# CloudEngineHub/FairyGen

Hardware: AMD Instinct MI355X
Metric: decoded frames/sec (sec/clip in config), Wan2.2-TI2V-5B 704x1280x121 @ 5 steps (higher is better)
Workload: dtype bf16

## Files before the change

### fairygen_amd/csrc/dit_elementwise.hip

```cpp
#include "common.h"
#include "rmsnorm_rope_row.h"

#ifndef FG_ROW_MIN_WAVES
#define FG_ROW_MIN_WAVES 4
#endif
#define FG_ROW_BOUNDS __launch_bounds__(256, FG_ROW_MIN_WAVES)

namespace {

__device__ __forceinline__ void row_moments(const Row& r, int C, int lane, float eps, float& mean, float& rstd) {
    const int nvec = C >> 3;
    float s = 0.f;
#pragma unroll
    for (int i = 0; i < kMaxVec; ++i)
#pragma unroll
        for (int j = 0; j < 8; ++j) s += r.v[i][j];
    mean = wave_sum(s) / (float)C;
    float q = 0.f;
#pragma unroll
    for (int i = 0; i < kMaxVec; ++i) {
        if (lane + i * 64 < nvec) {
#pragma unroll
            for (int j = 0; j < 8; ++j) {
                const float d = r.v[i][j] - mean;
                q += d * d;
            }
        }
    }
    const float var = wave_sum(q) / (float)C;
    rstd = 1.0f / sqrtf(var + eps);
}

__device__ __forceinline__ int64_t mod_row(int64_t row, int64_t mod_rows, int64_t first_rows) {
    return mod_rows == 1 ? 0 : (mod_rows == 2 ? (row < first_rows ? 0 : 1) : row);
}

template <int MODE>
__device__ __forceinline__ void norm_store(const Row& r, int C, int lane, float eps, const bf16* p0, const bf16* p1,
                                           bf16* out) {
    const int nvec = C >> 3;
    float mean, rstd;
    row_moments(r, C, lane, eps, mean, rstd);
#pragma unroll
    for (int i = 0; i < kMaxVec; ++i) {
        const int vi = lane + i * 64;
        if (vi < nvec) {
            const bf16x8 a = ld8(p0 + (int64_t)vi * 8);
            const bf16x8 b = ld8(p1 + (int64_t)vi * 8);
            float o[8];
#pragma unroll
            for (int j = 0; j < 8; ++j) {
                const float n = (r.v[i][j] - mean) * rstd;
                if (MODE == 0) {
                    const float y = rbf(n);
                    const float s1 = rbf(1.0f + (float)b[j]);
                    o[j] = rbf(y * s1) + (float)a[j];
                } else {
                    o[j] = n * (float)a[j] + (float)b[j];
                }
            }
            st8(out + (int64_t)vi * 8, o);
        }
    }
}

__device__ __forceinline__ uint32_t cvt2_fp8(float a, float b) {
    return (uint32_t)__builtin_amdgcn_cvt_pk_fp8_f32(a, b, 0, false) & 0xffffu;
}

template <int MODE, bool DUAL = false>
__device__ __forceinline__ void norm_store_fp8(Row& r, int C, int lane, float eps, const bf16* p0, const bf16* p1,
                                               uint8_t* out8, float* scale_out, float fp8_max, bf16* out16 = nullptr) {
    const int nvec = C >> 3;
    float mean, rstd;
    row_moments(r, C, lane, eps, mean, rstd);
    float amax = 0.f;
#pragma unroll
    for (int i = 0; i < kMaxVec; ++i) {
        const int vi = lane + i * 64;
        if (vi < nvec) {
            const bf16x8 a = ld8(p0 + (int64_t)vi * 8);
            const bf16x8 b = ld8(p1 + (int64_t)vi * 8);
#pragma unroll
            for (int j = 0; j < 8; ++j) {
                const float n = (r.v[i][j] - mean) * rstd;
                float o;
                if (MODE == 0) {
                    const float y = rbf(n);
                    const float s1 = rbf(1.0f + (float)b[j]);
                    o = rbf(y * s1) + (float)a[j];
                } else {
                    o = n * (float)a[j] + (float)b[j];
                }
                r.v[i][j] = rbf(o);
                amax = fmaxf(amax, fabsf(r.v[i][j]));
            }
            if (DUAL) st8(out16 + (int64_t)vi * 8, r.v[i]);
        }
    }
    amax = wave_max(amax);
    const float sc = fmaxf(rbf(amax / fp8_max), 1.0f);
    const float denom = sc + 1e-8f;
    if (lane == 0) *scale_out = sc;
#pragma unroll
    for (int i = 0; i < kMaxVec; ++i) {
        const int vi = lane + i * 64;
        if (vi < nvec) {
            u32x2 w;
            w[0] = cvt2_fp8(r.v[i][0] / denom, r.v[i][1] / denom) | (cvt2_fp8(r.v[i][2] / denom, r.v[i][3] / denom) << 16);
            w[1] = cvt2_fp8(r.v[i][4] / denom, r.v[i][5] / denom) | (cvt2_fp8(r.v[i][6] / denom, r.v[i][7] / denom) << 16);
            *reinterpret_cast<u32x2*>(out8 + (int64_t)vi * 8) = w;
        }
    }
}

__global__ FG_ROW_BOUNDS void ln_modulate_fp8_kernel(const bf16* __restrict__ x, const bf16* __restrict__ shift,
                                                     const bf16* __restrict__ scale, uint8_t* __restrict__ out8,
                                                     float* __restrict__ scale_out, int64_t rows, int C, float eps, int64_t mod_rows,
                                                     int64_t first_rows, int64_t mod_ld, float fp8_max) {
    const int lane = threadIdx.x & 63;
    const int64_t row = (int64_t)blockIdx.x * kRowsPerBlock + (threadIdx.x >> 6);
    if (row >= rows) return;
    Row r;
    load_row(x + row * C, C, lane, r);
    const int64_t m = mod_row(row, mod_rows, first_rows);
    norm_store_fp8<0>(r, C, lane, eps, shift + m * mod_ld, scale + m * mod_ld, out8 + row * C, scale_out + row, fp8_max);
}

template <int MODE>
__global__ FG_ROW_BOUNDS void ln_dual_kernel(const bf16* __restrict__ x, const bf16* __restrict__ p0, const bf16* __restrict__ p1,
                                             bf16* __restrict__ out, uint8_t* __restrict__ out8, float* __restrict__ scale_out,
                                             int64_t rows, int C, float eps, int64_t mod_rows, int64_t first_rows, int64_t mod_ld,
                                             float fp8_max) {
    const int lane = threadIdx.x & 63;
    const int64_t row = (int64_t)blockIdx.x * kRowsPerBlock + (threadIdx.x >> 6);
    if (row >= rows) return;
    Row r;
    load_row(x + row * C, C, lane, r);
    const int64_t m = MODE == 0 ? mod_row(row, mod_rows, first_rows) : 0;
    norm_store_fp8<MODE, true>(r, C, lane, eps, p0 + m * mod_ld, p1 + m * mod_ld, out8 + row * C, scale_out + row, fp8_max, out + row * C);
}

__global__ FG_ROW_BOUNDS void ln_modulate_kernel(const bf16* __restrict__ x, const bf16* __restrict__ shift,
                                                          const bf16* __restrict__ scale, bf16* __restrict__ out,
                                                          int64_t rows, int C, float eps, int64_t mod_rows,
                                                          int64_t first_rows, int64_t mod_ld) {
    const int lane = threadIdx.x & 63;
    const int64_t row = (int64_t)blockIdx.x * kRowsPerBlock + (threadIdx.x >> 6);
    if (row >= rows) return;
    Row r;
    load_row(x + row * C, C, lane, r);
    const int64_t m = mod_row(row, mod_rows, first_rows);
    norm_store<0>(r, C, lane, eps, shift + m * mod_ld, scale + m * mod_ld, out + row * C);
}

__global__ FG_ROW_BOUNDS void ln_affine_kernel(const bf16* __restrict__ x, const bf16* __restrict__ w,
                                                        const bf16* __restrict__ b, bf16* __restrict__ out,
                                                        int64_t rows, int C, float eps) {
    const int lane = threadIdx.x & 63;
    const int64_t row = (int64_t)blockIdx.x * kRowsPerBlock + (threadIdx.x >> 6);
    if (row >= rows) return;
    Row r;
    load_row(x + row * C, C, lane, r);
    norm_store<1>(r, C, lane, eps, w, b, out + row * C);
}

template <int MODE>
__global__ FG_ROW_BOUNDS void residual_kernel(const bf16* __restrict__ x, const bf16* __restrict__ y,
                                                       const bf16* __restrict__ gate, bf16* __restrict__ x_out,
                                                       const bf16* __restrict__ p0, const bf16* __restrict__ p1,
                                                       bf16* __restrict__ norm_out, int64_t rows, int C, float eps,
                                                       int64_t mod_rows, int64_t first_rows, int64_t mod_ld,
                                                       uint8_t* __restrict__ norm_fp8 = nullptr, float* __restrict__ norm_scale = nullptr,
                                                       float fp8_max = 0.f) {
    const int lane = threadIdx.x & 63;
    const int64_t row = (int64_t)blockIdx.x * kRowsPerBlock + (threadIdx.x >> 6);
    if (row >= rows) return;
    const int nvec = C >> 3;
    const int64_t m = mod_row(row, mod_rows, first_rows);
    Row r;
#pragma unroll
    for (int i = 0; i < kMaxVec; ++i) {
        const int vi = lane + i * 64;
        if (vi < nvec) {
            const bf16x8 xv = ld8(x + row * C + (int64_t)vi * 8);
            const bf16x8 yv = ld8(y + row * C + (int64_t)vi * 8);
            if (gate != nullptr) {
                const bf16x8 gv = ld8(gate + m * mod_ld + (int64_t)vi * 8);
#pragma unroll
                for (int j = 0; j < 8; ++j) r.v[i][j] = rbf((float)xv[j] + rbf((float)gv[j] * (float)yv[j]));
            } else {
#pragma unroll
                for (int j = 0; j < 8; ++j) r.v[i][j] = rbf((float)xv[j] + (float)yv[j]);
            }
            st8(x_out + row * C + (int64_t)vi * 8, r.v[i]);
        } else {
#pragma unroll
            for (int j = 0; j < 8; ++j) r.v[i][j] = 0.f;
        }
    }
    if (norm_fp8 != nullptr) {
        if (MODE == 0) norm_store_fp8<0>(r, C, lane, eps, p0 + m * mod_ld, p1 + m * mod_ld, norm_fp8 + row * C, norm_scale + row, fp8_max);
        if (MODE == 1) norm_store_fp8<1>(r, C, lane, eps, p0, p1, norm_fp8 + row * C, norm_scale + row, fp8_max);
        return;
    }
    if (MODE == 0) norm_store<0>(r, C, lane, eps, p0 + m * mod_ld, p1 + m * mod_ld, norm_out + row * C);
    if (MODE == 1) norm_store<1>(r, C, lane, eps, p0, p1, norm_out + row * C);
}

template <bool F32TAB, bool PLAIN = false>
__global__ FG_ROW_BOUNDS void rmsnorm_rope_kernel(const bf16* __restrict__ x, int64_t ldx,
                                                           const bf16* __restrict__ w, const void* __restrict__ ctv,
                                                           const void* __restrict__ stv, bf16* __restrict__ out,
                                                           int64_t rows, int C, int head_dim, float eps, int group_cols,
                                                           int64_t out_group_stride, int64_t out_ld) {
    const int lane = threadIdx.x & 63;
    const int64_t row = (int64_t)blockIdx.x * kRowsPerBlock + (threadIdx.x >> 6);
    if (row >= rows) return;
    Row r;
    load_row(x + row * ldx, C, lane, r);
    const int nvec = C >> 3;
    const RopeRow rr = rope_begin<F32TAB, PLAIN>(r, ctv, row, C, head_dim, eps, lane);
#pragma unroll
    for (int i = 0; i < kMaxVec; ++i) {
        const int vi = lane + i * 64;
        if (vi < nvec) {
            float o[8];
            rope_vec<F32TAB, PLAIN>(rr, r.v[i], ld8(w + (int64_t)vi * 8), ctv, stv, row, head_dim, vi, o);
            const int col = vi * 8, g = PLAIN ? 0 : col / group_cols;
            st8(out + g * out_group_stride + row * out_ld + (col - g * group_cols), o);
        }
    }
}

__global__ __launch_bounds__(256) void copy_groups_kernel(const bf16* __restrict__ src, int64_t sgs, int64_t sld,
                                                          bf16* __restrict__ dst, int64_t dgs, int64_t dld, int groups,
                                                          int64_t rows, int vec_per_row) {
    const int64_t total = (int64_t)groups * rows * vec_per_row;
    for (int64_t i = (int64_t)blockIdx.x * blockDim.x + threadIdx.x; i < total; i += (int64_t)gridDim.x * blockDim.x) {
        const int64_t rg = i / vec_per_row;
        const int v = (int)(i - rg * vec_per_row);
        const int64_t r = rg / groups;
        const int g = (int)(rg - r * groups);
        *reinterpret_cast<u32x4*>(dst + g * dgs + r * dld + v * 8) =
            *reinterpret_cast<const u32x4*>(src + g * sgs + r * sld + v * 8);
    }
}


template <int KIND>
__global__ __launch_bounds__(256) void act_kernel(const bf16* __restrict__ x, bf16* __restrict__ out, int64_t nvec) {
    for (int64_t i = (int64_t)blockIdx.x * blockDim.x + threadIdx.x; i < nvec; i += (int64_t)gridDim.x * blockDim.x) {
        const bf16x8 v = ld8(x + i * 8);
        float o[8];
#pragma unroll
        for (int j = 0; j < 8; ++j) o[j] = KIND == 0 ? silu_f((float)v[j]) : gelu_tanh_f((float)v[j]);
        st8(out + i * 8, o);
    }
}

__device__ __forceinline__ float cfg_euler_one(float lat, float p, float ng, bool has_nega, float cfg, float dsigma) {
    const float pred = has_nega ? rbf(ng + rbf(cfg * rbf(p - ng))) : p;
    return rbf(lat + rbf(pred * dsigma));
}

__global__ __launch_bounds__(256) void cfg_euler_kernel(const bf16* __restrict__ lat, const bf16* __restrict__ posi,
                                                        const bf16* __restrict__ nega, bf16* __restrict__ out,
                                                        int64_t n, float cfg, float dsigma) {
    for (int64_t i = (int64_t)blockIdx.x * blockDim.x + threadIdx.x; i < n; i += (int64_t)gridDim.x * blockDim.x)
        out[i] = (bf16)cfg_euler_one((float)lat[i], (float)posi[i], nega != nullptr ? (float)nega[i] : 0.0f, nega != nullptr, cfg, dsigma);
}

__global__ __launch_bounds__(256) void cfg_euler_dev_kernel(const bf16* lat, const bf16* __restrict__ posi, const bf16* __restrict__ nega,
                                                            bf16* out, int64_t n, int64_t nvec, float cfg,
                                                            const float* __restrict__ dsigma_table, const int* __restrict__ step,
                                                            const bf16* __restrict__ first, int64_t first_n, int64_t frame_stride) {
    const float dsigma = dsigma_table[*step];
    const bool has_nega = nega != nullptr;
    const int64_t tid = (int64_t)blockIdx.x * blockDim.x + threadIdx.x, nthreads = (int64_t)gridDim.x * blockDim.x;
    for (int64_t i = tid; i < nvec; i += nthreads) {
        const bf16x8 l = ld8(lat + i * 8), p = ld8(posi + i * 8);
        const bf16x8 g = has_nega ? ld8(nega + i * 8) : p;
        float o[8];
#pragma unroll
        for (int j = 0; j < 8; ++j) o[j] = cfg_euler_one((float)l[j], (float)p[j], (float)g[j], has_nega, cfg, dsigma);
        if (first != nullptr) {
            int64_t ch = (i * 8) / frame_stride, r = i * 8 - ch * frame_stride;
            if (r < first_n || r + 7 >= frame_stride) {
#pragma unroll
                for (int j = 0; j < 8; ++j) {
                    if (r < first_n) o[j] = (float)first[ch * first_n + r];
                    if (++r == frame_stride) { r = 0; ++ch; }
                }
            }
        }
        st8(out + i * 8, o);
    }
    for (int64_t i = nvec * 8 + tid; i < n; i += nthreads) {
        float o = cfg_euler_one((float)lat[i], (float)posi[i], has_nega ? (float)nega[i] : 0.0f, has_nega, cfg, dsigma);
        if (first != nullptr) {
            const int64_t ch = i / frame_stride, r = i - ch * frame_stride;
            if (r < first_n) o = (float)first[ch * first_n + r];
        }
        out[i] = (bf16)o;
    }
}

inline int check_rows(const char* fn, int64_t rows, int C, int64_t mod_rows, int64_t first_rows) {
    FG_CHECK_ARG(rows >= 0 && C > 0 && (C % 8) == 0 && C <= kMaxVec * 512, "%s: need C %% 8 == 0 and C <= %d (got rows=%lld C=%d)",
                 fn, kMaxVec * 512, (long long)rows, C);
    FG_CHECK_ARG(mod_rows == 1 || mod_rows == 2 || mod_rows == rows, "%s: mod_rows must be 1, 2 or rows (got %lld)", fn,
                 (long long)mod_rows);
    FG_CHECK_ARG(first_rows >= 0 && first_rows <= rows, "%s: first_rows out of range", fn);
    return FG_OK;
}

inline dim3 row_grid(int64_t rows) { return dim3((unsigned)((rows + kRowsPerBlock - 1) / kRowsPerBlock)); }

}

extern "C" {

int fg_ln_modulate_bf16(const void* x, const void* shift, const void* scale, void* out, int64_t rows, int C, float eps,
                        int64_t mod_rows, int64_t first_rows, int64_t mod_ld, fg_stream_t stream) {
    if (int e = check_rows("fg_ln_modulate_bf16", rows, C, mod_rows, first_rows)) return e;
    FG_CHECK_ARG(x && shift && scale && out, "fg_ln_modulate_bf16: null pointer");
    FG_CHECK_ARG(FG_ALIGNED16(x) && FG_ALIGNED16(shift) && FG_ALIGNED16(scale) && FG_ALIGNED16(out) && mod_ld % 8 == 0,
                 "fg_ln_modulate_bf16: pointers / mod_ld must be 16-byte aligned");
    if (rows == 0) return FG_OK;
    hipLaunchKernelGGL(ln_modulate_kernel, row_grid(rows), dim3(256), 0, (hipStream_t)stream, (const bf16*)x,
                       (const bf16*)shift, (const bf16*)scale, (bf16*)out, rows, C, eps, mod_rows, first_rows, mod_ld);
    return fg_launch_status("fg_ln_modulate_bf16");
}

int fg_ln_modulate_fp8_bf16(const void* x, const void* shift, const void* scale, void* out_fp8, float* out_scale, int64_t rows, int C,
                            float eps, int64_t mod_rows, int64_t first_rows, int64_t mod_ld, float fp8_max, fg_stream_t stream) {
    if (int e = check_rows("fg_ln_modulate_fp8_bf16", rows, C, mod_rows, first_rows)) return e;
    FG_CHECK_ARG(x && shift && scale && out_fp8 && out_scale, "fg_ln_modulate_fp8_bf16: null pointer");
    FG_CHECK_ARG(FG_ALIGNED16(x) && FG_ALIGNED16(shift) && FG_ALIGNED16(scale) && (((uintptr_t)out_fp8) & 7) == 0 && mod_ld % 8 == 0 &&
                     fp8_max > 0.f,
                 "fg_ln_modulate_fp8_bf16: pointers / mod_ld must be 16-byte aligned (out_fp8: 8), fp8_max positive");
    if (rows == 0) return FG_OK;
    hipLaunchKernelGGL(ln_modulate_fp8_kernel, row_grid(rows), dim3(256), 0, (hipStream_t)stream, (const bf16*)x, (const bf16*)shift,
                       (const bf16*)scale, (uint8_t*)out_fp8, out_scale, rows, C, eps, mod_rows, first_rows, mod_ld, fp8_max);
    return fg_launch_status("fg_ln_modulate_fp8_bf16");
}

int fg_ln_modulate_dual_bf16(const void* x, const void* shift, const void* scale, void* out, void* out_fp8, float* out_scale,
                             int64_t rows, int C, float eps, int64_t mod_rows, int64_t first_rows, int64_t mod_ld, float fp8_max,
                             fg_stream_t stream) {
    if (int e = check_rows("fg_ln_modulate_dual_bf16", rows, C, mod_rows, first_rows)) return e;
    FG_CHECK_ARG(x && shift && scale && out && out_fp8 && out_scale, "fg_ln_modulate_dual_bf16: null pointer");
    FG_CHECK_ARG(FG_ALIGNED16(x) && FG_ALIGNED16(shift) && FG_ALIGNED16(scale) && FG_ALIGNED16(out) && (((uintptr_t)out_fp8) & 7) == 0 &&
                     mod_ld % 8 == 0 && fp8_max > 0.f,
                 "fg_ln_modulate_dual_bf16: pointers / mod_ld must be 16-byte aligned (out_fp8: 8), fp8_max positive");
    if (rows == 0) return FG_OK;
    hipLaunchKernelGGL(ln_dual_kernel<0>, row_grid(rows), dim3(256), 0, (hipStream_t)stream, (const bf16*)x, (const bf16*)shift,
                       (const bf16*)scale, (bf16*)out, (uint8_t*)out_fp8, out_scale, rows, C, eps, mod_rows, first_rows, mod_ld, fp8_max);
    return fg_launch_status("fg_ln_modulate_dual_bf16");
}

int fg_ln_affine_dual_bf16(const void* x, const void* w, const void* b, void* out, void* out_fp8, float* out_scale, int64_t rows, int C,
                           float eps, float fp8_max, fg_stream_t stream) {
    if (int e = check_rows("fg_ln_affine_dual_bf16", rows, C, 1, 0)) return e;
    FG_CHECK_ARG(x && w && b && out && out_fp8 && out_scale, "fg_ln_affine_dual_bf16: null pointer");
    FG_CHECK_ARG(FG_ALIGNED16(x) && FG_ALIGNED16(w) && FG_ALIGNED16(b) && FG_ALIGNED16(out) && (((uintptr_t)out_fp8) & 7) == 0 &&
                     fp8_max > 0.f,
                 "fg_ln_affine_dual_bf16: pointers must be 16-byte aligned (out_fp8: 8), fp8_max positive");
    if (rows == 0) return FG_OK;
    hipLaunchKernelGGL(ln_dual_kernel<1>, row_grid(rows), dim3(256), 0, (hipStream_t)stream, (const bf16*)x, (const bf16*)w,
                       (const bf16*)b, (bf16*)out, (uint8_t*)out_fp8, out_scale, rows, C, eps, (int64_t)1, (int64_t)0, (int64_t)0, fp8_max);
    return fg_launch_status("fg_ln_affine_dual_bf16");
}

int fg_residual_ln_fp8_bf16(const void* x, const void* y, const void* gate, void* x_out, const void* p0, const void* p1,
                            void* norm_fp8, float* norm_scale, int mode, int64_t rows, int C, float eps, int64_t mod_rows,
                            int64_t first_rows, int64_t mod_ld, float fp8_max, fg_stream_t stream) {
    FG_CHECK_ARG(mode == 0 || mode == 1, "fg_residual_ln_fp8_bf16: mode must be 0 (modulate) or 1 (affine)");
    const bool need_mod = gate != nullptr || mode == 0;
    if (int e = check_rows("fg_residual_ln_fp8_bf16", rows, C, need_mod ? mod_rows : 1, need_mod ? first_rows : 0)) return e;
    FG_CHECK_ARG(x && y && x_out && p0 && p1 && norm_fp8 && norm_scale, "fg_residual_ln_fp8_bf16: null pointer");
    FG_CHECK_ARG(FG_ALIGNED16(x) && FG_ALIGNED16(y) && FG_ALIGNED16(gate) && FG_ALIGNED16(x_out) && FG_ALIGNED16(p0) &&
                     FG_ALIGNED16(p1) && (((uintptr_t)norm_fp8) & 7) == 0 && mod_ld % 8 == 0 && fp8_max > 0.f,
                 "fg_residual_ln_fp8_bf16: pointers / mod_ld must be 16-byte aligned (norm_fp8: 8), fp8_max positive");
    if (rows == 0) return FG_OK;
    if (!need_mod) { mod_rows = 1; first_rows = 0; }
    if (mode == 0)
        hipLaunchKernelGGL(residual_kernel<0>, row_grid(rows), dim3(256), 0, (hipStream_t)stream, (const bf16*)x,
                           (const bf16*)y, (const bf16*)gate, (bf16*)x_out, (const bf16*)p0, (const bf16*)p1,
                           (bf16*)nullptr, rows, C, eps, mod_rows, first_rows, mod_ld, (uint8_t*)norm_fp8, norm_scale, fp8_max);
    else
        hipLaunchKernelGGL(residual_kernel<1>, row_grid(rows), dim3(256), 0, (hipStream_t)stream, (const bf16*)x,
                           (const bf16*)y, (const bf16*)gate, (bf16*)x_out, (const bf16*)p0, (const bf16*)p1,
                           (bf16*)nullptr, rows, C, eps, mod_rows, first_rows, mod_ld, (uint8_t*)norm_fp8, norm_scale, fp8_max);
    return fg_launch_status("fg_residual_ln_fp8_bf16");
}

int fg_ln_affine_bf16(const void* x, const void* w, const void* b, void* out, int64_t rows, int C, float eps,
                      fg_stream_t stream) {
    if (int e = check_rows("fg_ln_affine_bf16", rows, C, 1, 0)) return e;
    FG_CHECK_ARG(x && w && b && out, "fg_ln_affine_bf16: null pointer");
    FG_CHECK_ARG(FG_ALIGNED16(x) && FG_ALIGNED16(w) && FG_ALIGNED16(b) && FG_ALIGNED16(out),
                 "fg_ln_affine_bf16: pointers must be 16-byte aligned");
    if (rows == 0) return FG_OK;
    hipLaunchKernelGGL(ln_affine_kernel, row_grid(rows), dim3(256), 0, (hipStream_t)stream, (const bf16*)x, (const bf16*)w,
                       (const bf16*)b, (bf16*)out, rows, C, eps);
    return fg_launch_status("fg_ln_affine_bf16");
}

int fg_gate_residual_bf16(const void* x, const void* y, const void* gate, void* out, int64_t rows, int C, int64_t mod_rows,
                          int64_t first_rows, int64_t mod_ld, fg_stream_t stream) {
    if (int e = check_rows("fg_gate_residual_bf16", rows, C, gate ? mod_rows : 1, gate ? first_rows : 0)) return e;
    FG_CHECK_ARG(x && y && out, "fg_gate_residual_bf16: null pointer");
    FG_CHECK_ARG(FG_ALIGNED16(x) && FG_ALIGNED16(y) && FG_ALIGNED16(gate) && FG_ALIGNED16(out) && mod_ld % 8 == 0,
                 "fg_gate_residual_bf16: pointers / mod_ld must be 16-byte aligned");
    if (rows == 0) return FG_OK;
    hipLaunchKernelGGL(residual_kernel<-1>, row_grid(rows), dim3(256), 0, (hipStream_t)stream, (const bf16*)x,
                       (const bf16*)y, (const bf16*)gate, (bf16*)out, (const bf16*)nullptr, (const bf16*)nullptr,
                       (bf16*)nullptr, rows, C, 0.f, gate ? mod_rows : 1, gate ? first_rows : 0, mod_ld);
    return fg_launch_status("fg_gate_residual_bf16");
}

int fg_residual_ln_bf16(const void* x, const void* y, const void* gate, void* x_out, const void* p0, const void* p1,
                        void* norm_out, int mode, int64_t rows, int C, float eps, int64_t mod_rows, int64_t first_rows,
                        int64_t mod_ld, fg_stream_t stream) {
    FG_CHECK_ARG(mode == 0 || mode == 1, "fg_residual_ln_bf16: mode must be 0 (modulate) or 1 (affine)");
    const bool need_mod = gate != nullptr || mode == 0;
    if (int e = check_rows("fg_residual_ln_bf16", rows, C, need_mod ? mod_rows : 1, need_mod ? first_rows : 0)) return e;
    FG_CHECK_ARG(x && y && x_out && p0 && p1 && norm_out, "fg_residual_ln_bf16: null pointer");
    FG_CHECK_ARG(FG_ALIGNED16(x) && FG_ALIGNED16(y) && FG_ALIGNED16(gate) && FG_ALIGNED16(x_out) && FG_ALIGNED16(p0) &&
                     FG_ALIGNED16(p1) && FG_ALIGNED16(norm_out) && mod_ld % 8 == 0,
                 "fg_residual_ln_bf16: pointers / mod_ld must be 16-byte aligned");
    if (rows == 0) return FG_OK;
    if (!need_mod) { mod_rows = 1; first_rows = 0; }
    if (mode == 0)
        hipLaunchKernelGGL(residual_kernel<0>, row_grid(rows), dim3(256), 0, (hipStream_t)stream, (const bf16*)x,
                           (const bf16*)y, (const bf16*)gate, (bf16*)x_out, (const bf16*)p0, (const bf16*)p1,
                           (bf16*)norm_out, rows, C, eps, mod_rows, first_rows, mod_ld);
    else
        hipLaunchKernelGGL(residual_kernel<1>, row_grid(rows), dim3(256), 0, (hipStream_t)stream, (const bf16*)x,
                           (const bf16*)y, (const bf16*)gate, (bf16*)x_out, (const bf16*)p0, (const bf16*)p1,
                           (bf16*)norm_out, rows, C, eps, mod_rows, first_rows, mod_ld);
    return fg_launch_status("fg_residual_ln_bf16");
}

int fg_rmsnorm_rope_bf16(const void* x, int64_t ldx, const void* weight, const void* cos_tab, const void* sin_tab,
                         int table_f32, void* out, int64_t rows, int C, int num_heads, float eps, fg_stream_t stream) {
    if (int e = check_rows("fg_rmsnorm_rope_bf16", rows, C, 1, 0)) return e;
    FG_CHECK_ARG(x && weight && out, "fg_rmsnorm_rope_bf16: null pointer");
    FG_CHECK_ARG(table_f32 ? (cos_tab != nullptr && sin_tab == nullptr) : ((cos_tab == nullptr) == (sin_tab == nullptr)),
                 "fg_rmsnorm_rope_bf16: fp64 mode takes both tables or neither, fp32 mode ONE interleaved table in cos_tab");
    FG_CHECK_ARG(num_heads > 0 && C % num_heads == 0 && (C / num_heads) % 8 == 0,
                 "fg_rmsnorm_rope_bf16: head_dim must be a multiple of 8");
    FG_CHECK_ARG(ldx >= C && ldx % 8 == 0 && FG_ALIGNED16(x) && FG_ALIGNED16(weight) && FG_ALIGNED16(out) &&
                     FG_ALIGNED16(cos_tab) && FG_ALIGNED16(sin_tab),
                 "fg_rmsnorm_rope_bf16: pointers / ldx must be 16-byte aligned");
    if (rows == 0) return FG_OK;
    const int hd = C / num_heads;
    const bool plain = (hd & (hd - 1)) == 0;
#define FG_ROPE_LAUNCH(TAB, PL)                                                                                                  \
    hipLaunchKernelGGL((rmsnorm_rope_kernel<TAB, PL>), row_grid(rows), dim3(256), 0, (hipStream_t)stream, (const bf16*)x, ldx,    \
                       (const bf16*)weight, cos_tab, sin_tab, (bf16*)out, rows, C, hd, eps, C, (int64_t)0, (int64_t)C)
    if (table_f32) { if (plain) FG_ROPE_LAUNCH(true, true); else FG_ROPE_LAUNCH(true, false); }
    else { if (plain) FG_ROPE_LAUNCH(false, true); else FG_ROPE_LAUNCH(false, false); }
#undef FG_ROPE_LAUNCH
    return fg_launch_status("fg_rmsnorm_rope_bf16");
}

int fg_rmsnorm_rope_grouped_bf16(const void* x, int64_t ldx, const void* weight, const void* cos_tab,
                                 const void* sin_tab, int table_f32, void* out, int64_t rows, int C, int num_heads, float eps,
                                 int group_cols, int64_t out_group_stride, int64_t out_ld, fg_stream_t stream) {
    if (int e = check_rows("fg_rmsnorm_rope_grouped_bf16", rows, C, 1, 0)) return e;
    FG_CHECK_ARG(x && weight && out, "fg_rmsnorm_rope_grouped_bf16: null pointer");
    FG_CHECK_ARG(table_f32 ? (cos_tab != nullptr && sin_tab == nullptr) : ((cos_tab == nullptr) == (sin_tab == nullptr)),
                 "fg_rmsnorm_rope_grouped_bf16: fp64 mode takes both tables or neither, fp32 mode ONE interleaved table in cos_tab");
    FG_CHECK_ARG(num_heads > 0 && C % num_heads == 0 && (C / num_heads) % 8 == 0,
                 "fg_rmsnorm_rope_grouped_bf16: head_dim must be a multiple of 8");
    FG_CHECK_ARG(group_cols > 0 && group_cols % 8 == 0 && C % group_cols == 0 && out_ld >= group_cols && out_ld % 8 == 0 &&
                     out_group_stride % 8 == 0 && out_group_stride >= 0,
                 "fg_rmsnorm_rope_grouped_bf16: group_cols must divide C; group_cols, out_ld, out_group_stride multiples of 8");
    FG_CHECK_ARG(ldx >= C && ldx % 8 == 0 && FG_ALIGNED16(x) && FG_ALIGNED16(weight) && FG_ALIGNED16(out) &&
                     FG_ALIGNED16(cos_tab) && FG_ALIGNED16(sin_tab),
                 "fg_rmsnorm_rope_grouped_bf16: pointers / ldx must be 16-byte aligned");
    if (rows == 0) return FG_OK;
    if (table_f32)
        hipLaunchKernelGGL((rmsnorm_rope_kernel<true, false>), row_grid(rows), dim3(256), 0, (hipStream_t)stream, (const bf16*)x, ldx,
                           (const bf16*)weight, cos_tab, sin_tab, (bf16*)out, rows, C, C / num_heads, eps, group_cols,
                           out_group_stride, out_ld);
    else
        hipLaunchKernelGGL((rmsnorm_rope_kernel<false, false>), row_grid(rows), dim3(256), 0, (hipStream_t)stream, (const bf16*)x, ldx,
                           (const bf16*)weight, cos_tab, sin_tab, (bf16*)out, rows, C, C / num_heads, eps, group_cols,
                           out_group_stride, out_ld);
    return fg_launch_status("fg_rmsnorm_rope_grouped_bf16");
}

int fg_copy_groups_bf16(const void* src, int64_t src_group_stride, int64_t src_ld, void* dst, int64_t dst_group_stride,
                        int64_t dst_ld, int groups, int64_t rows, int cols, fg_stream_t stream) {
    FG_CHECK_ARG(src && dst, "fg_copy_groups_bf16: null pointer");
    FG_CHECK_ARG(groups > 0 && rows >= 0 && cols > 0 && cols % 8 == 0, "fg_copy_groups_bf16: cols must be a positive multiple of 8");
    FG_CHECK_ARG(src_group_stride % 8 == 0 && src_ld % 8 == 0 && dst_group_stride % 8 == 0 && dst_ld % 8 == 0 &&
                     src_ld >= cols && dst_ld >= cols && FG_ALIGNED16(src) && FG_ALIGNED16(dst),
                 "fg_copy_groups_bf16: strides must be multiples of 8 elements, rows at least cols wide, pointers 16-byte aligned");
    if (rows == 0) return FG_OK;
    const int64_t total = (int64_t)groups * rows * (cols / 8);
    const unsigned grid = (unsigned)((total + 255) / 256 < 16384 ? (total + 255) / 256 : 16384);
    hipLaunchKernelGGL(copy_groups_kernel, dim3(grid), dim3(256), 0, (hipStream_t)stream, (const bf16*)src, src_group_stride,
                       src_ld, (bf16*)dst, dst_group_stride, dst_ld, groups, rows, cols / 8);
    return fg_launch_status("fg_copy_groups_bf16");
}

int fg_act_bf16(const void* x, void* out, int64_t n, int kind, fg_stream_t stream) {
    FG_CHECK_ARG(x && out && n >= 0 && n % 8 == 0, "fg_act_bf16: n must be a multiple of 8");
    FG_CHECK_ARG(kind == 0 || kind == 1, "fg_act_bf16: kind must be 0 (silu) or 1 (gelu_tanh)");
    FG_CHECK_ARG(FG_ALIGNED16(x) && FG_ALIGNED16(out), "fg_act_bf16: pointers must be 16-byte aligned");
    if (n == 0) return FG_OK;
    const int64_t nvec = n / 8;
    const unsigned grid = (unsigned)((nvec + 255) / 256 < 8192 ? (nvec + 255) / 256 : 8192);
    if (kind == 0)
        hipLaunchKernelGGL(act_kernel<0>, dim3(grid), dim3(256), 0, (hipStream_t)stream, (const bf16*)x, (bf16*)out, nvec);
    else
        hipLaunchKernelGGL(act_kernel<1>, dim3(grid), dim3(256), 0, (hipStream_t)stream, (const bf16*)x, (bf16*)out, nvec);
    return fg_launch_status("fg_act_bf16");
}

int fg_cfg_euler_bf16(const void* latents, const void* posi, const void* nega, void* out, int64_t n, float cfg_scale,
                      float dsigma, fg_stream_t stream) {
    FG_CHECK_ARG(latents && posi && out && n >= 0, "fg_cfg_euler_bf16: null pointer");
    if (n == 0) return FG_OK;
    const unsigned grid = (unsigned)((n + 255) / 256 < 4096 ? (n + 255) / 256 : 4096);
    hipLaunchKernelGGL(cfg_euler_kernel, dim3(grid), dim3(256), 0, (hipStream_t)stream, (const bf16*)latents,
                       (const bf16*)posi, (const bf16*)nega, (bf16*)out, n, cfg_scale, dsigma);
    return fg_launch_status("fg_cfg_euler_bf16");
}

int fg_cfg_euler_dev_bf16(const void* latents, const void* posi, const void* nega, void* out, int64_t n, float cfg_scale,
                          const float* dsigma_table, const int* step, const void* first, int64_t first_n, int64_t frame_stride,
                          fg_stream_t stream) {
    FG_CHECK_ARG(latents && posi && out && dsigma_table && step && n >= 0, "fg_cfg_euler_dev_bf16: null pointer");
    FG_CHECK_ARG((((uintptr_t)dsigma_table) & 3) == 0 && (((uintptr_t)step) & 3) == 0, "fg_cfg_euler_dev_bf16: dsigma_table / step must be 4-byte aligned");
    FG_CHECK_ARG(first == nullptr || (first_n > 0 && frame_stride >= first_n && n % frame_stride == 0),
                 "fg_cfg_euler_dev_bf16: with `first`, need 0 < first_n <= frame_stride and n a multiple of frame_stride (got n=%lld first_n=%lld "
                 "frame_stride=%lld)", (long long)n, (long long)first_n, (long long)frame_stride);
    if (n == 0) return FG_OK;
    const bool vec = FG_ALIGNED16(latents) && FG_ALIGNED16(posi) && FG_ALIGNED16(out) && (nega == nullptr || FG_ALIGNED16(nega));
    const int64_t nvec = vec ? n / 8 : 0;
    const int64_t work = nvec > n - nvec * 8 ? nvec : n - nvec * 8;
    const unsigned grid = (unsigned)((work + 255) / 256 < 4096 ? (work + 255) / 256 : 4096);
    hipLaunchKernelGGL(cfg_euler_dev_kernel, dim3(grid), dim3(256), 0, (hipStream_t)stream, (const bf16*)latents, (const bf16*)posi,
                       (const bf16*)nega, (bf16*)out, n, nvec, cfg_scale, dsigma_table, step, (const bf16*)first, first_n, frame_stride);
    return fg_launch_status("fg_cfg_euler_dev_bf16");
}

}
```

### fairygen_amd/csrc/rmsnorm_rope_row.h

```cpp
#pragma once
#include "common.h"

namespace {

constexpr int kMaxVec = 8;
constexpr int kRowsPerBlock = 4;

template <int NV>
struct RowT {
    float v[NV][8];
};
typedef RowT<kMaxVec> Row;

template <int NV>
__device__ __forceinline__ void load_row(const bf16* p, int C, int lane, RowT<NV>& r) {
    const int nvec = C >> 3;
#pragma unroll
    for (int i = 0; i < NV; ++i) {
        const int vi = lane + i * 64;
        if (vi < nvec) {
            bf16x8 t = *reinterpret_cast<const bf16x8*>(p + (int64_t)vi * 8);
#pragma unroll
            for (int j = 0; j < 8; ++j) r.v[i][j] = (float)t[j];
        } else {
#pragma unroll
            for (int j = 0; j < 8; ++j) r.v[i][j] = 0.f;
        }
    }
}

__device__ __forceinline__ bf16x8 ld8(const bf16* p) { return *reinterpret_cast<const bf16x8*>(p); }
__device__ __forceinline__ void st8(bf16* p, const float* f) {
    bf16x8 t;
#pragma unroll
    for (int j = 0; j < 8; ++j) t[j] = (bf16)f[j];
    *reinterpret_cast<bf16x8*>(p) = t;
}

struct RopeRow {
    float rinv;
    bool hoist;
    f32x4 h0, h1;
};

template <bool F32TAB, bool PLAIN, int NV>
__device__ __forceinline__ RopeRow rope_begin(const RowT<NV>& r, const void* ctv, int64_t row, int C, int head_dim, float eps, int lane) {
    RopeRow c;
    float q = 0.f;
#pragma unroll
    for (int i = 0; i < NV; ++i)
#pragma unroll
        for (int j = 0; j < 8; ++j) q += r.v[i][j] * r.v[i][j];
    const float ms = wave_sum(q) / (float)C;
    c.rinv = 1.0f / sqrtf(ms + eps);
    const int half = head_dim >> 1;
    c.hoist = F32TAB && ctv != nullptr && (512 % head_dim) == 0;
    c.h0 = f32x4{0.f, 0.f, 0.f, 0.f};
    c.h1 = f32x4{0.f, 0.f, 0.f, 0.f};
    if (c.hoist) {
        const int d_lane = PLAIN ? ((lane * 8) & (head_dim - 1)) : ((lane * 8) % head_dim);
        const f32x4* tp = reinterpret_cast<const f32x4*>(static_cast<const float*>(ctv) + (row * half + (d_lane >> 1)) * 2);
        c.h0 = tp[0];
        c.h1 = tp[1];
    }
    return c;
}

template <bool F32TAB, bool PLAIN>
__device__ __forceinline__ void rope_vec(const RopeRow& c, const float* rv, const bf16x8 wv, const void* ctv, const void* stv, int64_t row,
                                         int head_dim, int vi, float* o) {
    const int half = head_dim >> 1;
#pragma unroll
    for (int j = 0; j < 8; ++j) o[j] = rbf(rbf(rv[j] * c.rinv) * (float)wv[j]);
    if (ctv != nullptr) {
        const int d0 = PLAIN ? ((vi * 8) & (head_dim - 1)) : ((vi * 8) % head_dim);
        if (F32TAB) {
            f32x4 t0 = c.h0, t1 = c.h1;
            if (!c.hoist) {
                const f32x4* tp = reinterpret_cast<const f32x4*>(static_cast<const float*>(ctv) + (row * half + (d0 >> 1)) * 2);
                t0 = tp[0];
                t1 = tp[1];
            }
            const float cs[8] = {t0[0], t0[1], t0[2], t0[3], t1[0], t1[1], t1[2], t1[3]};
#pragma unroll
            for (int j = 0; j < 4; ++j) {
                const float a = o[2 * j], b = o[2 * j + 1], cc = cs[2 * j], sn = cs[2 * j + 1];
                o[2 * j] = rbf(__builtin_fmaf(a, cc, -(b * sn)));
                o[2 * j + 1] = rbf(__builtin_fmaf(a, sn, b * cc));
            }
        } else {
            const double* cp = static_cast<const double*>(ctv) + row * half + (d0 >> 1);
            const double* sp = static_cast<const double*>(stv) + row * half + (d0 >> 1);
#pragma unroll
            for (int j = 0; j < 4; ++j) {
                const double a = (double)o[2 * j], b = (double)o[2 * j + 1];
                const double cc = cp[j], sn = sp[j];
                o[2 * j] = (float)(bf16)(a * cc - b * sn);
                o[2 * j + 1] = (float)(bf16)(a * sn + b * cc);
            }
        }
    }
}

}
```

Before: 15.57.

## Add persistent row-walk kernels for LayerNorm and RMSNorm-RoPE with next-row prefetch

Adds persistent grid-stride kernels for rows with C in (2560, 3072], the Wan2.2-5B hidden size. Each wave walks several rows and issues the load of the next row before normalizing the current one. The modulation, affine and weight vectors stay in packed bf16 registers across rows and are reloaded only when the modulation row changes. This is meant to hide global-load latency and avoid reloading per-row parameters. In exchange it uses a fixed grid of CUs×3 blocks with higher register pressure, which may cut occupancy.

```diff
diff --git a/fairygen_amd/csrc/dit_elementwise.hip b/fairygen_amd/csrc/dit_elementwise.hip
--- a/fairygen_amd/csrc/dit_elementwise.hip
+++ b/fairygen_amd/csrc/dit_elementwise.hip
@@ -5,20 +5,23 @@
 #define FG_ROW_MIN_WAVES 4
 #endif
 #define FG_ROW_BOUNDS __launch_bounds__(256, FG_ROW_MIN_WAVES)
+#define FG_WALK_WAVES 3
+#define FG_WALK_BOUNDS __launch_bounds__(256, FG_WALK_WAVES)
 
 namespace {
 
-__device__ __forceinline__ void row_moments(const Row& r, int C, int lane, float eps, float& mean, float& rstd) {
+template <int NV>
+__device__ __forceinline__ void row_moments(const RowT<NV>& r, int C, int lane, float eps, float& mean, float& rstd) {
     const int nvec = C >> 3;
     float s = 0.f;
 #pragma unroll
-    for (int i = 0; i < kMaxVec; ++i)
+    for (int i = 0; i < NV; ++i)
 #pragma unroll
         for (int j = 0; j < 8; ++j) s += r.v[i][j];
     mean = wave_sum(s) / (float)C;
     float q = 0.f;
 #pragma unroll
-    for (int i = 0; i < kMaxVec; ++i) {
+    for (int i = 0; i < NV; ++i) {
         if (lane + i * 64 < nvec) {
 #pragma unroll
             for (int j = 0; j < 8; ++j) {
@@ -233,6 +236,142 @@
     }
 }
 
+constexpr int kWalkVec = 6;
+typedef RowT<kWalkVec> WalkRow;
+struct RawRow {
+    bf16x8 v[kWalkVec];
+};
+
+__device__ __forceinline__ void load_raw(const bf16* p, int nvec, int lane, RawRow& w) {
+#pragma unroll
+    for (int i = 0; i < kWalkVec; ++i) {
+        const int vi = lane + i * 64;
+        bf16x8 t;
+#pragma unroll
+        for (int j = 0; j < 8; ++j) t[j] = (bf16)0.f;
+        if (vi < nvec) t = ld8(p + (int64_t)vi * 8);
+        w.v[i] = t;
+    }
+}
+
+__device__ __forceinline__ void keep_packed(RawRow& w) {
+#pragma unroll
+    for (int i = 0; i < kWalkVec; ++i) asm volatile("" : "+v"(w.v[i]));
+}
+
+__device__ __forceinline__ void widen(const RawRow& w, WalkRow& r) {
+#pragma unroll
+    for (int i = 0; i < kWalkVec; ++i)
+#pragma unroll
+        for (int j = 0; j < 8; ++j) r.v[i][j] = (float)w.v[i][j];
+}
+
+template <int MODE>
+__device__ __forceinline__ void norm_store_held(const WalkRow& r, int C, int lane, float eps, const RawRow& pa, const RawRow& pb,
+                                                bf16* out) {
+    const int nvec = C >> 3;
+    float mean, rstd;
+    row_moments(r, C, lane, eps, mean, rstd);
+#pragma unroll
+    for (int i = 0; i < kWalkVec; ++i) {
+        const int vi = lane + i * 64;
+        if (vi < nvec) {
+            const bf16x8 a = pa.v[i];
+            const bf16x8 b = pb.v[i];
+            float o[8];
+#pragma unroll
+            for (int j = 0; j < 8; ++j) {
+                const float n = (r.v[i][j] - mean) * rstd;
+                if (MODE == 0) {
+                    const float y = rbf(n);
+                    const float s1 = (float)b[j];
+                    o[j] = rbf(y * s1) + (float)a[j];
+                } else {
+                    o[j] = n * (float)a[j] + (float)b[j];
+                }
+            }
+            st8(out + (int64_t)vi * 8, o);
+        }
+    }
+}
+
+template <int MODE>
+__global__ FG_WALK_BOUNDS void ln_walk_kernel(const bf16* __restrict__ x, const bf16* __restrict__ p0, const bf16* __restrict__ p1,
+                                             bf16* __restrict__ out, int64_t rows, int C, float eps, int64_t mod_rows,
+                                             int64_t first_rows, int64_t mod_ld) {
+    const int lane = threadIdx.x & 63, nvec = C >> 3;
+    const int64_t stride = (int64_t)gridDim.x * kRowsPerBlock;
+    int64_t row = (int64_t)blockIdx.x * kRowsPerBlock + (threadIdx.x >> 6);
+    if (row >= rows) return;
+    RawRow next, pa, pb;
+    load_raw(x + row * C, nvec, lane, next);
+    int64_t held = -1;
+    for (;;) {
+        WalkRow r;
+        widen(next, r);
+        const int64_t nrow = row + stride;
+        if (nrow < rows) load_raw(x + nrow * C, nvec, lane, next);
+        const int64_t m = MODE == 0 ? mod_row(row, mod_rows, first_rows) : 0;
+        if (m != held) {
+            load_raw(p0 + m * mod_ld, nvec, lane, pa);
+            load_raw(p1 + m * mod_ld, nvec, lane, pb);
+            if (MODE == 0) {
+#pragma unroll
+                for (int i = 0; i < kWalkVec; ++i)
+#pragma unroll
+                    for (int j = 0; j < 8; ++j) pb.v[i][j] = (bf16)(1.0f + (float)pb.v[i][j]);
+            }
+            held = m;
+        }
+        keep_packed(pa);
+        keep_packed(pb);
+        norm_store_held<MODE>(r, C, lane, eps, pa, pb, out + row * C);
+        if (nrow >= rows) return;
+        row = nrow;
+    }
+}
+
+template <bool F32TAB>
+__global__ FG_WALK_BOUNDS void rmsnorm_rope_walk_kernel(const bf16* __restrict__ x, int64_t ldx, const bf16* __restrict__ w,
+                                                       const void* __restrict__ ctv, const void* __restrict__ stv,
+                                                       bf16* __restrict__ out, int64_t rows, int C, int head_dim, float eps) {
+    const int lane = threadIdx.x & 63, nvec = C >> 3;
+    const int64_t stride = (int64_t)gridDim.x * kRowsPerBlock;
+    int64_t row = (int64_t)blockIdx.x * kRowsPerBlock + (threadIdx.x >> 6);
+    if (row >= rows) return;
+    RopeRow rr;
+    rr.hoist = F32TAB && ctv != nullptr && (512 % head_dim) == 0;
+    f32x4 n0 = f32x4{0.f, 0.f, 0.f, 0.f}, n1 = f32x4{0.f, 0.f, 0.f, 0.f};
+    RawRow next, wv;
+    load_raw(x + row * ldx, nvec, lane, next);
+    if (rr.hoist) rope_pairs<true>(ctv, row, head_dim, lane, n0, n1);
+    load_raw(w, nvec, lane, wv);
+    for (;;) {
+        WalkRow r;
+        widen(next, r);
+        rr.h0 = n0;
+        rr.h1 = n1;
+        const int64_t nrow = row + stride;
+        if (nrow < rows) {
+            load_raw(x + nrow * ldx, nvec, lane, next);
+            if (rr.hoist) rope_pairs<true>(ctv, nrow, head_dim, lane, n0, n1);
+        }
+        rr.rinv = rope_rinv(r, C, eps);
+        keep_packed(wv);
+#pragma unroll
+        for (int i = 0; i < kWalkVec; ++i) {
+            const int vi = lane + i * 64;
+            if (vi < nvec) {
+                float o[8];
+                rope_vec<F32TAB, true>(rr, r.v[i], wv.v[i], ctv, stv, row, head_dim, vi, o);
+                st8(out + row * C + (int64_t)vi * 8, o);
+            }
+        }
+        if (nrow >= rows) return;
+        row = nrow;
+    }
+}
+
 __global__ __launch_bounds__(256) void copy_groups_kernel(const bf16* __restrict__ src, int64_t sgs, int64_t sld,
                                                           bf16* __restrict__ dst, int64_t dgs, int64_t dld, int groups,
                                                           int64_t rows, int vec_per_row) {
@@ -317,6 +456,18 @@
 
 inline dim3 row_grid(int64_t rows) { return dim3((unsigned)((rows + kRowsPerBlock - 1) / kRowsPerBlock)); }
 
+inline int walk_grid() {
+    int dev = 0, cus = 0;
+    if (hipGetDevice(&dev) != hipSuccess || hipDeviceGetAttribute(&cus, hipDeviceAttributeMultiprocessorCount, dev) != hipSuccess || cus <= 0)
+        cus = 256;
+    return cus * FG_WALK_WAVES;
+}
+
+inline bool walks(int64_t rows, int C, int64_t mod_rows, bool plain_rows) {
+    return C > (kWalkVec - 1) * 512 && C <= kWalkVec * 512 && mod_rows <= 2 && plain_rows &&
+           rows > (int64_t)walk_grid() * kRowsPerBlock;
+}
+
 }
 
 extern "C" {
@@ -328,8 +479,12 @@
     FG_CHECK_ARG(FG_ALIGNED16(x) && FG_ALIGNED16(shift) && FG_ALIGNED16(scale) && FG_ALIGNED16(out) && mod_ld % 8 == 0,
                  "fg_ln_modulate_bf16: pointers / mod_ld must be 16-byte aligned");
     if (rows == 0) return FG_OK;
-    hipLaunchKernelGGL(ln_modulate_kernel, row_grid(rows), dim3(256), 0, (hipStream_t)stream, (const bf16*)x,
-                       (const bf16*)shift, (const bf16*)scale, (bf16*)out, rows, C, eps, mod_rows, first_rows, mod_ld);
+    if (walks(rows, C, mod_rows, true))
+        hipLaunchKernelGGL(ln_walk_kernel<0>, dim3(walk_grid()), dim3(256), 0, (hipStream_t)stream, (const bf16*)x,
+                           (const bf16*)shift, (const bf16*)scale, (bf16*)out, rows, C, eps, mod_rows, first_rows, mod_ld);
+    else
+        hipLaunchKernelGGL(ln_modulate_kernel, row_grid(rows), dim3(256), 0, (hipStream_t)stream, (const bf16*)x,
+                           (const bf16*)shift, (const bf16*)scale, (bf16*)out, rows, C, eps, mod_rows, first_rows, mod_ld);
     return fg_launch_status("fg_ln_modulate_bf16");
 }
 
@@ -403,8 +558,12 @@
     FG_CHECK_ARG(FG_ALIGNED16(x) && FG_ALIGNED16(w) && FG_ALIGNED16(b) && FG_ALIGNED16(out),
                  "fg_ln_affine_bf16: pointers must be 16-byte aligned");
     if (rows == 0) return FG_OK;
-    hipLaunchKernelGGL(ln_affine_kernel, row_grid(rows), dim3(256), 0, (hipStream_t)stream, (const bf16*)x, (const bf16*)w,
-                       (const bf16*)b, (bf16*)out, rows, C, eps);
+    if (walks(rows, C, 1, true))
+        hipLaunchKernelGGL(ln_walk_kernel<1>, dim3(walk_grid()), dim3(256), 0, (hipStream_t)stream, (const bf16*)x, (const bf16*)w,
+                           (const bf16*)b, (bf16*)out, rows, C, eps, (int64_t)1, (int64_t)0, (int64_t)0);
+    else
+        hipLaunchKernelGGL(ln_affine_kernel, row_grid(rows), dim3(256), 0, (hipStream_t)stream, (const bf16*)x, (const bf16*)w,
+                           (const bf16*)b, (bf16*)out, rows, C, eps);
     return fg_launch_status("fg_ln_affine_bf16");
 }
 
@@ -461,8 +620,13 @@
 #define FG_ROPE_LAUNCH(TAB, PL)                                                                                                  \
     hipLaunchKernelGGL((rmsnorm_rope_kernel<TAB, PL>), row_grid(rows), dim3(256), 0, (hipStream_t)stream, (const bf16*)x, ldx,    \
                        (const bf16*)weight, cos_tab, sin_tab, (bf16*)out, rows, C, hd, eps, C, (int64_t)0, (int64_t)C)
-    if (table_f32) { if (plain) FG_ROPE_LAUNCH(true, true); else FG_ROPE_LAUNCH(true, false); }
+#define FG_ROPE_WALK(TAB)                                                                                                        \
+    hipLaunchKernelGGL((rmsnorm_rope_walk_kernel<TAB>), dim3(walk_grid()), dim3(256), 0, (hipStream_t)stream, (const bf16*)x, ldx, \
+                       (const bf16*)weight, cos_tab, sin_tab, (bf16*)out, rows, C, hd, eps)
+    if (walks(rows, C, 1, plain)) { if (table_f32) FG_ROPE_WALK(true); else FG_ROPE_WALK(false); }
+    else if (table_f32) { if (plain) FG_ROPE_LAUNCH(true, true); else FG_ROPE_LAUNCH(true, false); }
     else { if (plain) FG_ROPE_LAUNCH(false, true); else FG_ROPE_LAUNCH(false, false); }
+#undef FG_ROPE_WALK
 #undef FG_ROPE_LAUNCH
     return fg_launch_status("fg_rmsnorm_rope_bf16");
 }
diff --git a/fairygen_amd/csrc/rmsnorm_rope_row.h b/fairygen_amd/csrc/rmsnorm_rope_row.h
--- a/fairygen_amd/csrc/rmsnorm_rope_row.h
+++ b/fairygen_amd/csrc/rmsnorm_rope_row.h
@@ -102,4 +102,24 @@
     }
 }
 
+template <int NV>
+__device__ __forceinline__ float rope_rinv(const RowT<NV>& r, int C, float eps) {
+    float q = 0.f;
+#pragma unroll
+    for (int i = 0; i < NV; ++i)
+#pragma unroll
+        for (int j = 0; j < 8; ++j) q += r.v[i][j] * r.v[i][j];
+    const float ms = wave_sum(q) / (float)C;
+    return 1.0f / sqrtf(ms + eps);
 }
+
+template <bool PLAIN>
+__device__ __forceinline__ void rope_pairs(const void* ctv, int64_t row, int head_dim, int lane, f32x4& h0, f32x4& h1) {
+    const int half = head_dim >> 1;
+    const int d_lane = PLAIN ? ((lane * 8) & (head_dim - 1)) : ((lane * 8) % head_dim);
+    const f32x4* tp = reinterpret_cast<const f32x4*>(static_cast<const float*>(ctv) + (row * half + (d_lane >> 1)) * 2);
+    h0 = tp[0];
+    h1 = tp[1];
+}
+
+}
```

After: 15.64 (median of 6 runs). About the same (+0.4%).
